# Stanford-ILIAD/PantheonRL

Measured on AMD Instinct MI355X. Metric: env-steps/sec (all agents) Overcooked-simple PPO self-play, higher is better.
Workload: dtype f32; 1 GPU; OvercookedMultiEnv-v0 layout=simple, PPO self-play (two independent PPO learners per GPU), synthetic (n_envs, n_steps, obs_dim) rollouts; n_envs=1024, n_steps=128, obs_dim=62, features=62, n_logits=6, batch_size=32768, n_epochs=10, agents_per_gpu=2, parallelism=2 agent(s) per gpu x1 gpu(s) = 2 learners (single process), launch_mode=graph, gemm_mode=2, action_masks=none, rollout=scripted, rollout_requested=scripted

## Files before the change

pantheonrl_amd/csrc/ph_abi.hip:

```cpp
#include <dlfcn.h>
#include <hip/hip_runtime.h>
#include <rccl/rccl.h>

#include <atomic>
#include <chrono>
#include <cmath>
#include <cstdio>
#include <cstdint>
#include <cstring>
#include <mutex>
#include <string>
#include <vector>

#include "ph_launch.h"
#include "ph_block.h"
#include "ph_arch.h"

namespace ph {

namespace {
struct LdsGrant {
  const void* kernel;
  int device;
  std::atomic<size_t> bytes;
// ... 84 lines not shown
  size_t grad_cap = 0;
  float* blocksq = nullptr;
  size_t blocksq_cap = 0;
  float* advstats = nullptr;
  size_t advstats_cap = 0;
  float* act_stage_host = nullptr;
  float* act_stage_dev = nullptr;
  size_t act_stage_cap = 0;
  unsigned int* act_done_host = nullptr;
  unsigned int* act_done_dev = nullptr;
  unsigned int act_seq = 0;
  unsigned int* fwd_host_done = nullptr;
  int joint_reward_rule = 0;
  int wimage_zeroed_for = 0;
  size_t wimage_cap = 0;
  bool exclusive = false;
  unsigned short* wimage = nullptr;
  double* advpart = nullptr;
  size_t advpart_cap = 0;
  int* perm_idx = nullptr;
  size_t perm_idx_cap = 0;
  int* perm_phys = nullptr;
  size_t perm_phys_cap = 0;
  uint4* ximg = nullptr;
  size_t ximg_cap = 0;
  uint4* rec_pi = nullptr;
  uint4* rec_vf = nullptr;
  size_t rec_cap = 0;
  uint4* rowrec = nullptr;
  size_t rowrec_cap = 0;
  unsigned long long* step_words = nullptr;
  size_t step_words_cap = 0;
  unsigned int* step_gen = nullptr;
  float* am_buf = nullptr;
  size_t am_buf_cap = 0;
  float* adap_extra = nullptr;
  size_t adap_extra_cap = 0;
  float* adap_loss = nullptr;
  size_t adap_loss_cap = 0;
  float* scalars = nullptr;
  int* stop_flag = nullptr;
  std::vector<SpecCache> specs;
  std::vector<hipGraphExec_t> graphs;
  bool capturing = false;
  hipEvent_t ev0 = nullptr, ev1 = nullptr;
  ph_p2p* p2p_dev = nullptr;
  ph_p2p p2p_host;
  bool p2p_valid = false;
  void* comm = nullptr;
  int comm_world = 1, comm_rank = 0;
  hipEvent_t ev_grad = nullptr;
  int num_cu = 256;
  int exchange_blocks_per_cu = 0;
  unsigned long long* rng_epoch = nullptr;
  long long* prof = nullptr;
  struct ModWs {
    float* act = nullptr;
    size_t act_cap = 0;
    int* maps = nullptr;
    ph_spec spec;
    ph_modular mod;
    bool maps_valid = false;
    float* kl_sum = nullptr;
    int* scratch = nullptr;
  } mw;
};
// ... 382 lines not shown
  hipDeviceProp_t prop;
  PH_HIP(hipGetDeviceProperties(&prop, device));
  if (std::strncmp(prop.gcnArchName, "gfx950", 6) != 0)
    return fail(std::string("device is ") + prop.gcnArchName + ", this library is built for gfx950 (MI355X) only");
  ph_ctx* c = new ph_ctx();
  c->device = device;
  c->num_cu = prop.multiProcessorCount;
  if (hipMalloc((void**)&c->scalars, 4 * sizeof(float)) != hipSuccess ||
      hipMalloc((void**)&c->stop_flag, sizeof(int)) != hipSuccess) {
    delete c;
    return fail("hipMalloc(ctx scalars) failed");
  }
  (void)hipMemset(c->scalars, 0, 4 * sizeof(float));
  (void)hipMemset(c->stop_flag, 0, sizeof(int));
  (void)hipEventCreate(&c->ev0);
  (void)hipEventCreate(&c->ev1);
  *out = c;
  return 0;
}

int ph_ctx_destroy(ph_ctx* ctx) {
  DevGuard dev_guard(ctx);
  if (!ctx) return 0;
  (void)hipStreamSynchronize(ctx->stream);
  for (auto g : ctx->graphs)
    if (g) (void)hipGraphExecDestroy(g);
  for (auto& s : ctx->specs) {
    if (s.obs_off) (void)hipFree(s.obs_off);
    if (s.slab_map) (void)hipFree(s.slab_map);
    if (s.slab_map_split) (void)hipFree(s.slab_map_split);
    if (s.wimage_map) (void)hipFree(s.wimage_map);
    if (s.act_off) (void)hipFree(s.act_off);
  }
  void* ptrs[] = {ctx->wimage, ctx->mw.act, ctx->mw.maps, ctx->mw.kl_sum, ctx->mw.scratch, ctx->advpart, ctx->p2p_dev, ctx->slabs, ctx->statpart, ctx->grad, ctx->blocksq, ctx->advstats, ctx->perm_idx, ctx->perm_phys, ctx->ximg, ctx->rec_pi, ctx->rec_vf, ctx->rowrec, ctx->step_words, ctx->step_gen, ctx->scalars, ctx->stop_flag,
                  ctx->adap_extra, ctx->adap_loss, ctx->am_buf};
  for (void* p : ptrs)
    if (p) (void)hipFree(p);
  if (ctx->act_stage_host) (void)hipHostFree(ctx->act_stage_host);
  if (ctx->act_done_host) (void)hipHostFree(ctx->act_done_host);
  if (ctx->ev0) (void)hipEventDestroy(ctx->ev0);
  if (ctx->ev1) (void)hipEventDestroy(ctx->ev1);
  if (ctx->ev_grad) (void)hipEventDestroy(ctx->ev_grad);
  (void)ph_comm_destroy(ctx);
  delete ctx;
  return 0;
}

int ph_ctx_set_joint_reward_rule(ph_ctx* ctx, int rule) {
  if (!ctx) return fail("null ctx");
  if (rule != PH_JOINT_MATCH_BONUS && rule != PH_JOINT_RPS) return fail("ph_ctx_set_joint_reward_rule: unknown rule");
  ctx->joint_reward_rule = rule;
  return 0;
}

int ph_ctx_set_stream(ph_ctx* ctx, void* hip_stream) {
  DevGuard dev_guard(ctx);
  if (!ctx) return fail("null ctx");
  ctx->stream = (hipStream_t)hip_stream;
  return 0;
}

int ph_ctx_sync(ph_ctx* ctx) {
  DevGuard dev_guard(ctx);
  if (!ctx) return fail("null ctx");
  PH_HIP(hipStreamSynchronize(ctx->stream));
  return 0;
}
// ... 1279 lines not shown
    ctx->rec_cap = n_rec;
  }
  PH_HIP(ph::launch_obs_planes(rb->observations, (int)rows, nd.D, nd.F, ph::grad_fast_fold(nd) ? 1 : 0, ctx->ximg, rb->advantages,
                               rb->log_probs, rb->actions, rb->returns, rb->values, ctx->rowrec, ctx->stream));
  return 0;
}
void fill_adv_records(ph::AdvStatArgs& aa, const ph_ctx* ctx, const ph::NetDims& nd, const ph_rollout* rb) {
  aa.rec_pi_out = nd.split == 1 ? ctx->rec_pi : nullptr;
  aa.rec_vf_out = nd.split == 1 ? ctx->rec_vf : nullptr;
  aa.rowrec = (nd.split == 1 && rb->advantages && rb->log_probs && rb->actions && rb->returns && rb->values) ? ctx->rowrec : nullptr;
  aa.rb_logp = rb->log_probs;
  aa.rb_act = rb->actions;
  aa.rb_ret = rb->returns;
  aa.rb_val = rb->values;
}


void select_gemm(ph::NetDims& nd, int gemm_mode) {
  nd.split = (gemm_mode == 2 && nd.slab_map_split != nullptr) ? nd.split_kind : 0;
  if (nd.split) nd.slab_map = nd.slab_map_split;
}

int slab_len_of(const ph::NetDims& nd) { return nd.split ? nd.slab_len_split : (nd.slab_map ? 2 * ph::RS_NET : nd.lay.P); }

int ensure_train_ws(ph_ctx* ctx, int P, int slab_len, int nwg_max, int n_mb_total, size_t n_idx = 0, size_t n_phys = 0) {
  if (n_phys && ensure(ctx, ctx->perm_phys, ctx->perm_phys_cap, n_phys)) return 1;
  if (ensure(ctx, ctx->slabs, ctx->slabs_cap, (size_t)nwg_max * slab_len)) return 1;
  if (ensure(ctx, ctx->statpart, ctx->statpart_cap, (size_t)2 * nwg_max * ph::NSTATP)) return 1;
  if (ensure(ctx, ctx->grad, ctx->grad_cap, (size_t)P)) return 1;
  if (ensure(ctx, ctx->blocksq, ctx->blocksq_cap, (size_t)ph::reduce_blocks(slab_len))) return 1;
  if (ensure(ctx, ctx->advstats, ctx->advstats_cap, (size_t)n_mb_total * 2)) return 1;
  if (ensure(ctx, ctx->advpart, ctx->advpart_cap, (size_t)n_mb_total * 2 * ph::ADV_SPLIT)) return 1;
  if (n_idx && ensure(ctx, ctx->perm_idx, ctx->perm_idx_cap, n_idx)) return 1;
  const size_t n_words = (size_t)ph::reduce_blocks(slab_len) + 1;
  if (n_words > ctx->step_words_cap) {
    if (ensure(ctx, ctx->step_words, ctx->step_words_cap, n_words)) return 1;
    PH_HIP(hipMemsetAsync(ctx->step_words, 0, n_words * sizeof(unsigned long long), ctx->stream));
  }
  if (!ctx->step_gen) {
    if (ctx->capturing) return fail("workspace would grow inside graph capture: run the same call once outside capture first");
    PH_HIP(hipMalloc((void**)&ctx->step_gen, 4 * sizeof(unsigned int)));
    PH_HIP(hipMemsetAsync(ctx->step_gen, 0, 4 * sizeof(unsigned int), ctx->stream));
  }
  return 0;
}

bool step_fused_wanted(const ph_ctx* ctx, int slab_len, bool alone) {
  return alone && ctx->exclusive && ctx->step_words && ctx->step_gen &&
         ph::step_fused_fits(ph::reduce_blocks(slab_len), slab_len, ctx->num_cu);
}

}

namespace {

struct TrainPlan {
  int alone = 1;
  ph_ctx* ctx;
  ph::NetDims nd;
  const ph_opt_state* opt;
  const ph_rollout* rb;
  const ph_ppo_hyper* hp;
  const int* perms;
  unsigned long long perm_seed;
  float* stats;
  int n_epochs, batch_size, gemm_mode, N, n_mb, P;
  uint32_t hb;
  const ph_adap_loss* adap = nullptr;
  bool arch = false;
  ph::ArchDims arch_dims;
};

int adap_check(ph_ctx* ctx, const ph::NetDims& nd, const ph_adap_loss* ad, const char* who) {
  const std::string w(who);
  if (nd.obs_kind != PH_SPACE_BOX) return fail(w + ": the context term needs Box observations (observation ++ context)");
  if (ad->context_size <= 0 || ad->context_size >= nd.F) return fail(w + ": context_size must be in (0, observation length)");
  if (ad->num_context_samples < 2 || ad->num_context_samples > ph::ADAP_ROWS)
    return fail(w + ": num_context_samples must be in [2, 16]");
  if (ad->num_state_samples <= 0) return fail(w + ": num_state_samples must be positive");
  if (ad->sampler < PH_CTX_L2 || ad->sampler > PH_CTX_NATURAL_NUMBERS) return fail(w + ": unknown context sampler");
  if (ad->sampler == PH_CTX_NATURAL_NUMBERS && ad->context_size != 1)
    return fail(w + ": the natural_numbers sampler draws (num, 1) contexts: context_size must be 1");
// ... 117 lines not shown
  g.perm_seed = t.perm_seed;
  g.perm_epoch = w.ep;
  g.epoch = ctx->rng_epoch;
  g.mb_start = w.start;
  g.nb = w.nb;
  g.advstats = ctx->advstats + 2 * (size_t)mbi;
  g.ntiles = pl.ntiles;
  *pl_out = pl;
  if (t.arch) PH_HIP(ph::launch_arch_grad(g, t.arch_dims, pl.nwg, t.gemm_mode, ctx->stream));
  else PH_HIP(ph::launch_ppo_grad(g, pl.nwg, t.gemm_mode, ctx->stream));
  return 0;
}

void fill_step_args(const TrainPlan& t, int mbi, const MbPlan& pl, ph::ReduceArgs& r, ph::AdamArgs& ad) {
  ph_ctx* ctx = t.ctx;
  float* stats_out = t.stats ? t.stats + (size_t)mbi * PH_NSTAT : nullptr;
  r = reduce_args(ctx, t.hp, t.opt, t.P, slab_len_of(t.nd), t.nd.slab_map, pl.nwg, pl.nb, ctx->grad, stats_out);
  r.wide = t.alone && ctx->exclusive;
  ad = adam_args(ctx, t.hp, t.opt, t.P, slab_len_of(t.nd), stats_out, t.nd.split ? ctx->wimage : nullptr, t.nd.wimage_map);
}

int train_launch_step(const TrainPlan& t, int mbi, const MbPlan& pl) {
  ph_ctx* ctx = t.ctx;
  hipStream_t s = ctx->stream;
  ph::ReduceArgs r;
  ph::AdamArgs ad;
  fill_step_args(t, mbi, pl, r, ad);
  if (t.adap) {
    const MbWalk w = minibatch_walk(ctx, t.perms, t.N, t.n_mb, t.batch_size, mbi);
    if (adap_launch(ctx, t.nd, t.opt->params, t.rb, t.adap, w.idx, w.nb, mbi, &r)) return 1;
  }
  if (step_fused_wanted(ctx, slab_len_of(t.nd), t.alone != 0)) {
    PH_HIP(ph::launch_ppo_step(r, ad, ctx->step_words, ctx->step_gen, ctx->step_gen + 1, STEP_WAIT_TICKS, s));
  } else {
    PH_HIP(ph::launch_ppo_reduce(r, s));
    PH_HIP(ph::launch_ppo_adam(ad, s));
  }
  return 0;
}

}

namespace {
int train_run(const char* who, ph_ctx* ctx, const ph_spec* spec, const ph_opt_state* opt, const ph_rollout* rb,
              const ph_ppo_hyper* hp, int n_epochs, int batch_size, const int* perms, unsigned long long perm_seed, float* stats,
              int gemm_mode, const ph_adap_loss* adap, const ph_arch* arch = nullptr) {
  TrainPlan t;
  if (train_prepare(who, t, ctx, spec, opt, rb, hp, n_epochs, batch_size, perms, perm_seed, stats, gemm_mode, adap != nullptr, arch))
    return 1;
  if (adap && t.nd.gauss) return fail("ph_adap_train: the context term is written for the categorical heads");
  if (adap && adap_check(ctx, t.nd, adap, "ph_adap_train")) return 1;
  t.adap = adap;
  for (int mbi = 0; mbi < n_epochs * t.n_mb; ++mbi) {
    MbPlan pl;
    if (train_launch_grad(t, mbi, &pl)) return 1;
    if (train_launch_step(t, mbi, pl)) return 1;
  }
  return 0;
}
}

int ph_ppo_train(ph_ctx* ctx, const ph_spec* spec, const ph_opt_state* opt, const ph_rollout* rb,
                 const ph_ppo_hyper* hp, int n_epochs, int batch_size, const int* perms,
                 unsigned long long perm_seed, float* stats, int gemm_mode) {
  DevGuard dev_guard(ctx);
  return train_run("ph_ppo_train", ctx, spec, opt, rb, hp, n_epochs, batch_size, perms, perm_seed, stats, gemm_mode, nullptr);
// ... 1041 lines not shown
```

pantheonrl_amd/csrc/ph_launch.h:

```cpp
#pragma once
#include "ph_device.h"

namespace ph {

__host__ __device__ inline unsigned p2p_stamp32(unsigned long long epoch, int T, int t) {
  return (unsigned)(epoch * (unsigned long long)T + (unsigned long long)t + 1ull);
}

__device__ __forceinline__ void p2p_note_timeout(unsigned long long* error, int kind, int t, unsigned long long index,
                                                 unsigned long long want, unsigned long long seen) {
  if (atomicAdd(error, 1ull) == 0ull) {
    error[1] = (unsigned long long)(unsigned)kind | ((unsigned long long)(unsigned)(t & 0xffffff) << 8) | (index << 32);
    error[2] = want;
    error[3] = seen;
  }
}

__device__ __forceinline__ void poll_backoff(int& polls) {
  if (polls < 16) __builtin_amdgcn_s_sleep(2);
  else if (polls < 64) __builtin_amdgcn_s_sleep(16);
  else __builtin_amdgcn_s_sleep(127);
  ++polls;
}

// ... 168 lines not shown
  const float* statpart;
  int nstatpart;
  float* stats_out;
  int nb;
  float ent_coef, vf_coef, target_kl;
  int* stop_flag;
  int* step;
  float* scalars;
  const float* extra = nullptr;
  int n_extra = 0, extra_len = 0, extra_cut = 0, extra_lo = 0, extra_hi = 0;
  const float* extra_loss = nullptr;
  float extra_norm = 0.f;
  float extra_coef = 0.f;
  float* extra_loss_out = nullptr;
  int wide = 0;
};

struct AdamArgs {
  float* params;
  float* m;
  float* v;
  const float* grad;
  const float* blocksq;
  int nblk, P;
  const int* step;
  const float* scalars;
  int* stop_flag;
  float lr, beta1, beta2, eps, max_norm;
  float* stats_out;
  unsigned short* wimage;
  const int* wimage_map;
};

struct StepArgs {
  ReduceArgs r;
  AdamArgs ad;
  unsigned long long* words = nullptr;
  unsigned int* gen = nullptr;
  unsigned long long timeout = 0;
  unsigned int* sweep_error = nullptr;
};

size_t fwd_lds_bytes(int R, int Lp);
size_t grad_lds_bytes(int R, int Lp, int onehot_D, int nchunk);
hipError_t launch_policy_fwd(const FwdArgs& a, int gemm_mode, hipStream_t s);
hipError_t launch_policy_fwd_multi(const FwdMulti& m, int n_agents, hipStream_t s);
hipError_t launch_fix_illegal(int* actions, const unsigned char* mask, int n, int L, hipStream_t s);
hipError_t launch_gae(const float* rew, const float* val, const float* es, const float* lv, const float* dn, float* adv,
                      float* ret, int T, int E, double gamma, double lam, int mode, hipStream_t s);
hipError_t launch_buffer_add(float* d_obs, float* d_act, float* d_rew, float* d_es, float* d_val, float* d_lp,
                             const float* obs, const float* act, const float* es, const float* val, const float* lp,
                             int E, int D, int A, hipStream_t s);
hipError_t launch_buffer_compact(const ph_rollout& src, const ph_rollout& dst, const int* cols, int n, int D, int A,
                                 hipStream_t s);
hipError_t launch_reward_add_ragged(float* rewards, const int* pos_env, const float* reward, const unsigned char* mask,
                                    int T, int E, hipStream_t s);
hipError_t launch_ragged_advance(int* pos_env, const unsigned char* mask, int T, int E, hipStream_t s);
hipError_t launch_liar_obs(const int* hands, const int* history, const int* nmoves, const unsigned char* is_ego,
                           const unsigned char* active, float* obs_out, int n, hipStream_t s);
hipError_t launch_liar_reset(int* hands, int* history, int* nmoves, const unsigned char* reset_mask,
                             unsigned char* ego_first, unsigned long long seed, unsigned long long counter,
                             const unsigned long long* epoch, float probegostart, int n, hipStream_t s);
hipError_t launch_reward_add(float* rew_row, const float* reward, const unsigned char* env_mask, int E, hipStream_t s);
hipError_t launch_reward_add_const(float* rew_row, float reward, int E, hipStream_t s);
hipError_t launch_reward_add_joint(float* rew_row, const float* base, const int* joint, int E, int n_seats, int seat,
                                   const int* partner_seat, float bonus, int rule, hipStream_t s);
hipError_t launch_framestack_push(float* stack, const float* obs, const unsigned char* reset_mask,
                                  const float* default_obs, int n, int D, int nf, hipStream_t s);
hipError_t launch_roundrobin_env_step(const int* joint, int* partnerid, const float* base, const float* done, float* reward_out,
                                      int* alt_action_out, float* next_block, int block_ld, int n_partners, float bonus, int n,
                                      hipStream_t s);
hipError_t launch_rps_step(const int* ego_act, const int* alt_act, float* ego_rew, float* alt_rew, int n, hipStream_t s);
hipError_t launch_liar_step(const int* hands, int* history, int* nmoves, const int* actions, const unsigned char* is_ego,
// ... 117 lines not shown
  const int* actions;
  int* act_dst;
};
hipError_t launch_rr_send_block(const RRSend& a, int n_partners, hipStream_t s);
hipError_t launch_rr_env_step(const RREnvStep& a, hipStream_t s);
hipError_t launch_rr_partner_pre(const RRPartnerStep& a, hipStream_t s);
hipError_t launch_rr_partner_post(const RRPartnerStep& a, hipStream_t s);
constexpr int RS_NET = 8960;
constexpr int RS_W2 = 0, RS_W1 = 4096, RS_B1 = 8192, RS_B2 = 8256, RS_HW = 8320, RS_HB = 8832;
bool grad_fast_eligible(const NetDims& nd);
bool grad_uses_reg_slabs(const NetDims& nd);
bool grad_fast_fold(const NetDims& nd);
void grad_slab_map(const ph_layout& lay, int* map , bool fold);
void grad_plan(const NetDims& nd, int nb, int num_cu, int* ntiles, int* nwg);
hipError_t launch_ppo_grad_fast(const GradArgs& a, int nwg, int gemm_mode, hipStream_t s);
bool grad_split_eligible(const NetDims& nd);
constexpr int WIMG_PLANE = 64 * 8;
constexpr int WIMG_ELEMS = 2 * 4 * 3 * 2 * 3 * WIMG_PLANE;
void grad_weight_image_map(const ph_layout& lay, bool fold, int* map );
hipError_t launch_weight_image(const float* params, unsigned short* image, const int* map, int P, hipStream_t s);
hipError_t launch_weight_image_check(const float* params, const unsigned short* image, const int* map, int P, int* mismatches,
                                     hipStream_t s);
void grad_slab_map_split(const ph_layout& lay, int* map , bool fold);
hipError_t launch_ppo_grad_split(const GradArgs& a, int nwg, hipStream_t s);
hipError_t launch_adv_stats(const AdvStatArgs& a, int n_total, hipStream_t s);
constexpr int XIMG_ROW_U4 = 24;
hipError_t launch_obs_planes(const float* obs, int n, int D, int F, int fold, uint4* image, const float* adv, const float* logp,
                             const float* act, const float* ret, const float* val, uint4* rowrec, hipStream_t s);
hipError_t launch_ppo_reduce(const ReduceArgs& a, hipStream_t s);
int reduce_blocks(int slab_len);
bool step_fused_fits(int nblk, int slab_len, int num_cu);
hipError_t launch_ppo_step(const ReduceArgs& r, const AdamArgs& ad, unsigned long long* words, unsigned int* gen,
                           unsigned int* sweep_error, unsigned long long timeout, hipStream_t st);
hipError_t launch_ppo_adam(const AdamArgs& a, hipStream_t s);
bool grad_split_oh_eligible(const NetDims& nd);
int grad_split_oh_slab_len(const NetDims& nd);
int grad_split_oh_wimage_elems(const NetDims& nd);
void grad_weight_image_map_oh(const ph_layout& lay, int nch, int* map );
void grad_slab_map_split_oh(const ph_layout& lay, int nch, int* map );
hipError_t launch_ppo_grad_split_oh(const GradArgs& a, int nwg, hipStream_t s);
hipError_t launch_set_int(int* p, int v, hipStream_t s);
size_t bc_train_lds_bytes(int F, int L, int P, int A);
hipError_t launch_bc_train(const NetDims& nd, const ph_bc_layout& lay, float* params, float* adam_m, float* adam_v, int* step,
                           const float* obs, const float* acts, const int* order, int N, int batch, int n_epochs,
                           int max_batches, const ph_bc_hyper& hp, float* stats, hipStream_t s);
hipError_t launch_bc_forward(const NetDims& nd, const ph_bc_layout& lay, const float* params, const float* obs, int n,
                             const unsigned char* mask, const float* uniforms, const float* given, uint64_t seed,
                             uint64_t counter, int deterministic, int* act_i32, float* values, float* logp, float* entropy,
                             float* logits, hipStream_t s);
hipError_t launch_epoch_advance(unsigned long long* p, hipStream_t s);

struct TowerArgs {
  int nb, ntiles;
  const float* x;
  int x_ld;
  int F;
  const int* obs_off;
  const int* idx;
  int T, E;
  const float *W1, *b1, *W2, *b2, *hW, *hb;
  int head;
  int L;
  float* h2_out;
  float* head_out;
  const float* dhead;
  const float* ext0;
// ... 66 lines not shown
```

pantheonrl_amd/csrc/ph_ppo.hip:

```cpp
#include "ph_launch.h"
#include "ph_split.h"
#include "ph_step.h"

namespace ph {


template <int N>
__device__ __forceinline__ float lds_colsum(const float* p, int stride, float s) {
#pragma unroll
  for (int r0 = 0; r0 < N; r0 += 16) {
    float t[16];
#pragma unroll
    for (int i = 0; i < 16; ++i) t[i] = p[(r0 + i) * stride];
    __builtin_amdgcn_sched_barrier(0);
#pragma unroll
    for (int i = 0; i < 16; ++i) s += t[i];
  }
  return s;
}
template <int N>
__device__ __forceinline__ float lds_coldot(const float* p, int stride, const float* q, int qstride, float s) {
#pragma unroll
  for (int r0 = 0; r0 < N; r0 += 16) {
    float t[16], u[16];
// ... 931 lines not shown
int reduce_blocks(int slab_len) { return (slab_len + RED_PARAMS - 1) / RED_PARAMS; }
static int reduce_vec(int slab_len, int exclusive) { return (slab_len % 4 == 0 && exclusive) ? 4 : (slab_len % 2 == 0 ? 2 : 1); }
bool step_fused_fits(int nblk, int slab_len, int num_cu) {
  if (nblk + 1 > 64 * 16) return false;
  static int per_cu[3] = {-1, -1, -1};
  const int vec = reduce_vec(slab_len, 1);
  int& v = per_cu[vec == 4 ? 2 : vec - 1];
  if (v < 0) {
    int api = 0;
    const void* fn = vec == 4 ? (const void*)ppo_step_kernel<4> : vec == 2 ? (const void*)ppo_step_kernel<2> : (const void*)ppo_step_kernel<1>;
    hipError_t e = hipOccupancyMaxActiveBlocksPerMultiprocessor(&api, fn, RED_PARAMS * 4, 0);
    v = (e == hipSuccess && api > 1) ? api - 1 : 0;
  }
  return (long long)v * num_cu >= (long long)nblk + 1;
}
hipError_t launch_ppo_step(const ReduceArgs& r, const AdamArgs& ad, unsigned long long* words, unsigned int* gen,
                           unsigned int* sweep_error, unsigned long long timeout, hipStream_t st) {
  StepArgs s;
  s.r = r;
  s.ad = ad;
  s.words = words;
  s.gen = gen;
  s.timeout = timeout;
  s.sweep_error = sweep_error;
  const int nblk = reduce_blocks(r.slab_len);
  if ((unsigned long long)r.nslab * (unsigned long long)r.slab_len * sizeof(float) >= (1ull << 32)) return hipErrorInvalidValue;
  switch (reduce_vec(r.slab_len, 1)) {
    case 4: hipLaunchKernelGGL(ppo_step_kernel<4>, dim3(nblk + 1), dim3(RED_PARAMS * 4), 0, st, s); break;
    case 2: hipLaunchKernelGGL(ppo_step_kernel<2>, dim3(nblk + 1), dim3(RED_PARAMS * 4), 0, st, s); break;
    default: hipLaunchKernelGGL(ppo_step_kernel<1>, dim3(nblk + 1), dim3(RED_PARAMS * 4), 0, st, s); break;
  }
  return hipGetLastError();
}
hipError_t launch_ppo_reduce(const ReduceArgs& a, hipStream_t s) {
  const dim3 grid(reduce_blocks(a.slab_len) + 1), block(RED_PARAMS * 4);
  if ((unsigned long long)a.nslab * (unsigned long long)a.slab_len * sizeof(float) >= (1ull << 32)) return hipErrorInvalidValue;
  switch (reduce_vec(a.slab_len, a.wide)) {
    case 4: hipLaunchKernelGGL(ppo_reduce_kernel<4>, grid, block, 0, s, a); break;
    case 2: hipLaunchKernelGGL(ppo_reduce_kernel<2>, grid, block, 0, s, a); break;
    default: hipLaunchKernelGGL(ppo_reduce_kernel<1>, grid, block, 0, s, a); break;
  }
  return hipGetLastError();
}

__global__ __launch_bounds__(256) void ppo_adam_kernel(AdamArgs a) {
  __shared__ float sh[4];
  __shared__ AdamScalars ks;
  const int tid = threadIdx.x;
  const int p = blockIdx.x * blockDim.x + tid;
  const bool live = p < a.P;
  float gr = 0.f, m0 = 0.f, v0 = 0.f, p0 = 0.f;
  int i0 = -1, i1 = -1;
  if (live) {
    gr = a.grad[p];
    m0 = a.m[p];
    v0 = a.v[p];
    p0 = a.params[p];
    if (a.wimage) {
      i0 = a.wimage_map[2 * p];
      i1 = a.wimage_map[2 * p + 1];
    }
  }
  if (a.scalars[1] == 0.f) {
    if (blockIdx.x == 0 && tid == 0 && a.scalars[2] != 0.f) *a.stop_flag = 1;
    return;
  }
  const int step = (tid == 0) ? *a.step : 0;
  float q = 0.f;
  {
    float x[4];
    for (int k0 = tid; k0 < a.nblk; k0 += 4 * 256) {
#pragma unroll
      for (int u = 0; u < 4; ++u) x[u] = (k0 + 256 * u < a.nblk) ? a.blocksq[k0 + 256 * u] : 0.f;
#pragma unroll
      for (int u = 0; u < 4; ++u)
        if (k0 + 256 * u < a.nblk) q += x[u];
    }
  }
  for (int off = 32; off > 0; off >>= 1) q += __shfl_down(q, off, 64);
  if ((tid & 63) == 0) sh[tid >> 6] = q;
  __syncthreads();
  if (tid == 0) {
    const float total = sqrtf((sh[0] + sh[1]) + (sh[2] + sh[3]));
    ks = adam_scalars(total, a.max_norm, step, a.lr, a.beta1, a.beta2);
    if (blockIdx.x == 0 && a.stats_out) a.stats_out[6] = total;
  }
  __syncthreads();
  if (!live) return;
  const AdamScalars k = ks;
  float m, v;
  const float pn = adam_apply(gr, k, a.beta1, a.beta2, a.eps, m0, v0, p0, &m, &v);
  a.m[p] = m;
  a.v[p] = v;
  a.params[p] = pn;
  if (a.wimage) wimage_put_at(a.wimage, i0, i1, pn);
}

__global__ __launch_bounds__(256) void weight_image_kernel(const float* params, unsigned short* image, const int* map, int P) {
  const int p = blockIdx.x * blockDim.x + threadIdx.x;
  if (p < P) wimage_put(image, map, p, params[p]);
}
__global__ __launch_bounds__(256) void weight_image_check_kernel(const float* params, const unsigned short* image, const int* map, int P,
                                                                 int* mismatches) {
  const int p = blockIdx.x * blockDim.x + threadIdx.x;
  if (p >= P) return;
  __bf16 h, m, l;
  split1(params[p], h, m, l);
  const unsigned short want[3] = {__builtin_bit_cast(unsigned short, h), __builtin_bit_cast(unsigned short, m),
                                  __builtin_bit_cast(unsigned short, l)};
  int bad = 0;
  for (int k = 0; k < 2; ++k) {
    const int pos = map[2 * p + k];
    if (pos < 0) continue;
    for (int q = 0; q < 3; ++q) bad += image[pos + q * WIMG_PLANE] != want[q];
  }
  if (bad) atomicAdd(mismatches, bad);
}
// ... 27 lines not shown
```

pantheonrl_amd/csrc/ph_step.h:

```cpp
#pragma once
#include "ph_launch.h"
#include "ph_split.h"

namespace ph {

constexpr int RED_PARAMS = 64, RED_SUB = 16, RED_SHIFT = 6;

struct AdamScalars {
  float coef, ss, bc2s;
};
__device__ __forceinline__ AdamScalars adam_scalars(float total_norm, float max_norm, int step, float lr, float beta1, float beta2) {
  AdamScalars k;
  const float cc = max_norm / (total_norm + 1e-6f);
  k.coef = cc < 1.0f ? cc : 1.0f;
  const double t = (double)step;
  const double bc1 = 1.0 - pow((double)beta1, t);
  const double bc2 = 1.0 - pow((double)beta2, t);
  k.ss = (float)((double)lr / bc1);
  k.bc2s = (float)sqrt(bc2);
  return k;
}
__device__ __forceinline__ float adam_apply(float grad, const AdamScalars& k, float beta1, float beta2, float eps, float m0, float v0,
                                            float p0, float* m_out, float* v_out) {
#pragma clang fp contract(off)
// ... 188 lines not shown
    stop = (a.target_kl >= 0.f) && (kl > 1.5f * a.target_kl);
    if (bump_step && !stop && a.step) *a.step += 1;
    a.scalars[0] = kl;
    a.scalars[1] = stop ? 0.f : 1.f;
    a.scalars[2] = stop ? 1.f : 0.f;
    if (a.stats_out) {
      a.stats_out[0] = pl_;
      a.stats_out[1] = vl;
      a.stats_out[2] = el;
      a.stats_out[3] = cf;
      a.stats_out[4] = kl;
      a.stats_out[5] = pl_ + a.ent_coef * el + a.vf_coef * vl;
      a.stats_out[6] = 0.f;
      a.stats_out[7] = stop ? 0.f : 1.f;
    }
    if (a.n_extra > 0) {
      float raw = 0.f;
      for (int k0 = 0; k0 < a.n_extra; k0 += 16) {
        float x[16];
#pragma unroll
        for (int u = 0; u < 16; ++u) x[u] = (k0 + u < a.n_extra) ? a.extra_loss[k0 + u] : 0.f;
#pragma unroll
        for (int u = 0; u < 16; ++u)
          if (k0 + u < a.n_extra) raw += x[u];
      }
      raw *= a.extra_norm;
      if (a.extra_loss_out) *a.extra_loss_out = raw;
      if (a.stats_out) a.stats_out[5] += a.extra_coef * raw;
    }
  }
  return stop;
}

__device__ __forceinline__ void step_finish(const StepArgs& s, int nblk, unsigned tag, int step_new, int lane, bool first, float g,
                                            int dst, float m0, float v0, float p0, int i0, int i1) {
  const ReduceArgs& a = s.r;
  const AdamArgs& ad = s.ad;
  AdamScalars k = adam_scalars(0.f, ad.max_norm, step_new, ad.lr, ad.beta1, ad.beta2);
  constexpr int MAXW = 16;
  float qv[MAXW];
  bool ok = false;
  const long long t0 = wall_clock64();
  while (true) {
    bool all = true;
#pragma unroll
    for (int i = 0; i < MAXW; ++i) {
      const int k = lane + 64 * i;
      qv[i] = 0.f;
      if (k <= nblk) {
        const unsigned long long w = __hip_atomic_load(s.words + k, __ATOMIC_RELAXED, __HIP_MEMORY_SCOPE_AGENT);
        all = all && ((unsigned)(w >> 32) == tag);
        qv[i] = __uint_as_float((unsigned)w);
      }
    }
    if (__all(all)) { ok = true; break; }
    if ((unsigned long long)(wall_clock64() - t0) > s.timeout) break;
    __builtin_amdgcn_s_sleep(4);
  }
  if (!ok) {
    if (lane == 0) {
      atomicAdd(s.sweep_error, 1u);
      if (first && a.stats_out) a.stats_out[7] = -1.f;
    }
    return;
  }
  int stop_i = 0;
#pragma unroll
  for (int i = 0; i < MAXW; ++i)
    if (lane + 64 * i == nblk) stop_i = __float_as_int(qv[i]) & 1;
  const bool stop = __any(stop_i != 0);
  float shv[4];
#pragma unroll
  for (int v = 0; v < 4; ++v) {
    float q = 0.f;
#pragma unroll
    for (int i = v; i < MAXW; i += 4)
      if (lane + 64 * i < nblk) q += qv[i];
    for (int off = 32; off > 0; off >>= 1) q += __shfl_down(q, off, 64);
    shv[v] = __shfl(q, 0, 64);
  }
  const float total = sqrtf((shv[0] + shv[1]) + (shv[2] + shv[3]));
  if (first && lane == 0) {
    if (!stop && ad.step) *const_cast<int*>(ad.step) = step_new;
    if (stop) *a.stop_flag = 1;
    *s.gen = tag;
    if (!stop && a.stats_out) a.stats_out[6] = total;
  }
  if (stop || dst < 0) return;
  {
    const float cc = ad.max_norm / (total + 1e-6f);
    k.coef = cc < 1.0f ? cc : 1.0f;
  }
  const int p = dst;
  float m, v;
  const float pn = adam_apply(g, k, ad.beta1, ad.beta2, ad.eps, m0, v0, p0, &m, &v);
  ad.m[p] = m;
  ad.v[p] = v;
  ad.params[p] = pn;
  if (ad.wimage) wimage_put_at(ad.wimage, i0, i1, pn);
}


__device__ __forceinline__ void step_stopped(const ReduceArgs& a) {
  const int tid = threadIdx.x;
  if (tid < PH_NSTAT && a.stats_out) a.stats_out[tid] = 0.f;
  if (tid == 0) {
    a.scalars[1] = 0.f;
    a.scalars[2] = 0.f;
  }
}
__device__ __forceinline__ bool step_refused(const ReduceArgs& a, int blk, int stopped, unsigned err) {
  if (err != 0u) {
    if (blk == 0 && threadIdx.x == 0 && a.stats_out) a.stats_out[7] = -1.f;
    return true;
// ... 13 lines not shown
  if (blk == nblk) {
    if (step_refused(a, blk, stopped, err)) return;
    const bool stop = reduce_statistics<COH>(a, part, means, false);
    if (tid == 0)
      __hip_atomic_store(s.words + nblk, ((unsigned long long)tag << 32) | (stop ? 1ull : 0ull), __ATOMIC_RELAXED, __HIP_MEMORY_SCOPE_AGENT);
    return;
  }
  const int dst = reduce_dst(a, blk);
  float m0 = 0.f, v0 = 0.f, p0 = 0.f;
  int i0 = -1, i1 = -1;
  if (dst >= 0) {
    m0 = ad.m[dst];
    v0 = ad.v[dst];
    p0 = ad.params[dst];
    if (ad.wimage) {
      i0 = ad.wimage_map[2 * dst];
      i1 = ad.wimage_map[2 * dst + 1];
    }
  }
  const float g = reduce_positions<VEC, COH>(a, gsum, dst, blk);
  if (step_refused(a, blk, stopped, err)) return;
  if (tid < 64) {
    float q = g * g;
    for (int off = 32; off > 0; off >>= 1) q += __shfl_down(q, off, 64);
    if (tid == 0)
      __hip_atomic_store(s.words + blk, ((unsigned long long)tag << 32) | (unsigned long long)__float_as_uint(q), __ATOMIC_RELAXED,
                         __HIP_MEMORY_SCOPE_AGENT);
  }
  if (tid >= 64) return;
  step_finish(s, nblk, tag, step_new, tid, blk == 0, g, dst, m0, v0, p0, i0, i1);
}


__host__ __device__ inline int reduce_blocks_of(int slab_len) { return (slab_len + RED_PARAMS - 1) / RED_PARAMS; }

}
```

pantheonrl_amd/ppo.py:

```python
from __future__ import annotations

import ctypes as C
import os
import io
import json
import time
import zipfile
from collections import deque
from typing import Sequence, Any, Dict, Optional, Tuple

import numpy as np
import torch as th

from . import _native as nat
from . import spaces as sp
from .logger import Logger, configure_logger

HID = nat.PH_HIDDEN


def _require_cuda(device) -> th.device:
    dev = th.device("cuda" if device in (None, "auto") else device)
    if dev.type != "cuda":
        raise nat.NativeError(
# ... 637 lines not shown
        prog = getattr(self, "_current_progress_remaining", 1.0)
        h.learning_rate, h.clip_range = self._schedule(self.learning_rate, prog), self._schedule(self.clip_range, prog)
        h.clip_range_vf = -1.0 if self.clip_range_vf is None else self._schedule(self.clip_range_vf, prog)
        h.ent_coef, h.vf_coef, h.max_grad_norm = float(self.ent_coef), float(self.vf_coef), float(self.max_grad_norm)
        h.target_kl = -1.0 if self.target_kl is None else float(self.target_kl)
        h.normalize_advantage = int(bool(self.normalize_advantage))
        h.adam_beta1, h.adam_beta2, h.adam_eps = 0.9, 0.999, 1e-5
        return h

    def train(self, perms: Optional[np.ndarray] = None, sync_stats: bool = True) -> None:
        rb, pol = self.rollout_buffer, self.policy
        N = rb.buffer_size * rb.n_envs
        n_mb = (N + self.batch_size - 1) // self.batch_size
        perm_t = None
        if perms is None and not self.device_permutations:
            perms = np.stack([np.random.permutation(N) for _ in range(self.n_epochs)])
        if perms is not None:
            perm_t = th.as_tensor(np.ascontiguousarray(perms, dtype=np.int32)).to(self.device)
            assert perm_t.shape == (self.n_epochs, N)
        stats = getattr(self, "_stats_dev", None)
        if stats is None or stats.shape[0] != self.n_epochs * n_mb:
            stats = th.zeros((self.n_epochs * n_mb, nat.PH_NSTAT), dtype=th.float32, device=self.device)
        opt = nat.PhOptState()
        opt.params, opt.adam_m, opt.adam_v = pol.params.data_ptr(), pol.adam_m.data_ptr(), pol.adam_v.data_ptr()
        opt.step = pol.opt_step.data_ptr()
        hp = self.hyper()
        pol._bind()
        self.permutation_seed += 1
        self._train_native(pol, opt, rb, hp, perm_t, stats)
        self._n_updates += self.n_epochs
        self._stats_dev = stats
        if sync_stats:
            st = stats.cpu().numpy()
            expired = pol.ctx.step_errors() if pol.ctx.exclusive_hint else 0
            seen, self._step_errors_seen = getattr(self, "_step_errors_seen", 0), expired
            if (st[:, 7] < 0).any() or expired > seen:
                raise nat.NativeError("PPO.train: a wait of the one-launch optimizer step expired (is the device really this "
                                      "learner's alone? ph_set_exclusive_device): the update was applied only in part")
            self.last_train_stats = st
            applied = st[:, 7] > 0
            n_used = int(applied.sum()) + (1 if not applied.all() else 0)
            used = st[:max(n_used, 1)]
            lg = self.logger
            ret = rb.returns.flatten()
            var_y = float(ret.var(unbiased=False))
            ev = float("nan") if var_y == 0 else 1.0 - float((ret - rb.values.flatten()).var(unbiased=False)) / var_y
            lg.record("train/explained_variance", ev)
            lg.record("train/entropy_loss", float(used[:, 2].mean()))
            lg.record("train/policy_gradient_loss", float(used[:, 0].mean()))
            lg.record("train/value_loss", float(used[:, 1].mean()))
            lg.record("train/approx_kl", float(used[((len(used) - 1) // n_mb) * n_mb:, 4].mean()))
            lg.record("train/clip_fraction", float(used[:, 3].mean()))
            lg.record("train/loss", float(used[-1, 5]))
            lg.record("train/n_updates", self._n_updates, exclude="tensorboard")
            lg.record("train/clip_range", float(hp.clip_range))
            lg.record("train/learning_rate", float(hp.learning_rate))

    def _train_native(self, pol, opt, rb, hp, perm_t, stats) -> None:
        if isinstance(pol, ArchActorCriticPolicy):
            nat.check(pol.ctx.lib.ph_arch_train(pol.ctx.handle, C.byref(pol.spec), C.byref(pol.arch), C.byref(opt),
                                                C.byref(rb.c_struct()), C.byref(hp), int(self.n_epochs), int(self.batch_size),
                                                nat.ptr(perm_t), int(self.permutation_seed), stats.data_ptr(), int(pol.gemm_mode)))
            return
        if not getattr(pol, "gaussian_head", False):
            require_mlp_kernels(pol, "PPO.train")
        nat.check(pol.ctx.lib.ph_ppo_train(pol.ctx.handle, C.byref(pol.spec), C.byref(opt), C.byref(rb.c_struct()),
                                           C.byref(hp), int(self.n_epochs), int(self.batch_size), nat.ptr(perm_t),
                                           int(self.permutation_seed), stats.data_ptr(), int(pol.gemm_mode)))

    def _train_call(self, keep: list) -> "nat.PhTrainCall":
        rb, pol = self.rollout_buffer, self.policy
# ... 221 lines not shown
```

Measured before the change: 119.2 million agent-steps/s.

## Fuse gradient reduce and Adam into one ticket-ordered launch for shared devices

Adds a single-launch optimizer step for the case where the fused step is not allowed, i.e. two learners share the GPU. Blocks take tickets from an atomic counter: ticket 0 computes statistics, the next tickets reduce gradient slabs and publish tagged per-parameter entries, and the remaining tickets spin until their entries and the norm words are ready, then apply Adam. Ordering by ticket means waiting blocks only depend on blocks that were already scheduled, so it is safe without exclusive residency. This saves a kernel launch and the inter-kernel gap per minibatch, at the cost of spin-wait polling, extra atomics and a per-parameter entries buffer.

```diff
diff --git a/pantheonrl_amd/csrc/ph_abi.hip b/pantheonrl_amd/csrc/ph_abi.hip
--- a/pantheonrl_amd/csrc/ph_abi.hip
+++ b/pantheonrl_amd/csrc/ph_abi.hip
@@ -140,6 +140,8 @@
   unsigned long long* step_words = nullptr;
   size_t step_words_cap = 0;
   unsigned int* step_gen = nullptr;
+  unsigned long long* step_entries = nullptr;
+  size_t step_entries_cap = 0;
   float* am_buf = nullptr;
   size_t am_buf_cap = 0;
   float* adap_extra = nullptr;
@@ -588,7 +590,7 @@
     if (s.wimage_map) (void)hipFree(s.wimage_map);
     if (s.act_off) (void)hipFree(s.act_off);
   }
-  void* ptrs[] = {ctx->wimage, ctx->mw.act, ctx->mw.maps, ctx->mw.kl_sum, ctx->mw.scratch, ctx->advpart, ctx->p2p_dev, ctx->slabs, ctx->statpart, ctx->grad, ctx->blocksq, ctx->advstats, ctx->perm_idx, ctx->perm_phys, ctx->ximg, ctx->rec_pi, ctx->rec_vf, ctx->rowrec, ctx->step_words, ctx->step_gen, ctx->scalars, ctx->stop_flag,
+  void* ptrs[] = {ctx->wimage, ctx->mw.act, ctx->mw.maps, ctx->mw.kl_sum, ctx->mw.scratch, ctx->advpart, ctx->p2p_dev, ctx->slabs, ctx->statpart, ctx->grad, ctx->blocksq, ctx->advstats, ctx->perm_idx, ctx->perm_phys, ctx->ximg, ctx->rec_pi, ctx->rec_vf, ctx->rowrec, ctx->step_words, ctx->step_entries, ctx->step_gen, ctx->scalars, ctx->stop_flag,
                   ctx->adap_extra, ctx->adap_loss, ctx->am_buf};
   for (void* p : ptrs)
     if (p) (void)hipFree(p);
@@ -1934,10 +1936,14 @@
   if (ensure(ctx, ctx->advstats, ctx->advstats_cap, (size_t)n_mb_total * 2)) return 1;
   if (ensure(ctx, ctx->advpart, ctx->advpart_cap, (size_t)n_mb_total * 2 * ph::ADV_SPLIT)) return 1;
   if (n_idx && ensure(ctx, ctx->perm_idx, ctx->perm_idx_cap, n_idx)) return 1;
-  const size_t n_words = (size_t)ph::reduce_blocks(slab_len) + 1;
+  const size_t n_words = std::max((size_t)ph::reduce_blocks(slab_len) + 1, (size_t)64 * ph::STEP_MAXW);
   if (n_words > ctx->step_words_cap) {
     if (ensure(ctx, ctx->step_words, ctx->step_words_cap, n_words)) return 1;
     PH_HIP(hipMemsetAsync(ctx->step_words, 0, n_words * sizeof(unsigned long long), ctx->stream));
+  }
+  if ((size_t)P > ctx->step_entries_cap) {
+    if (ensure(ctx, ctx->step_entries, ctx->step_entries_cap, (size_t)P)) return 1;
+    PH_HIP(hipMemsetAsync(ctx->step_entries, 0, (size_t)P * sizeof(unsigned long long), ctx->stream));
   }
   if (!ctx->step_gen) {
     if (ctx->capturing) return fail("workspace would grow inside graph capture: run the same call once outside capture first");
@@ -1950,6 +1956,14 @@
 bool step_fused_wanted(const ph_ctx* ctx, int slab_len, bool alone) {
   return alone && ctx->exclusive && ctx->step_words && ctx->step_gen &&
          ph::step_fused_fits(ph::reduce_blocks(slab_len), slab_len, ctx->num_cu);
+}
+
+bool step_ordered_wanted(const ph_ctx* ctx, int slab_len, int P) {
+  static const bool on = [] {
+    const char* e = getenv("PH_STEP_ORDERED");
+    return !(e && e[0] == '0');
+  }();
+  return on && ctx->step_words && ctx->step_entries && ctx->step_gen && ph::step_ordered_fits(ph::reduce_blocks(slab_len), P);
 }
 
 }
@@ -2133,6 +2147,9 @@
   }
   if (step_fused_wanted(ctx, slab_len_of(t.nd), t.alone != 0)) {
     PH_HIP(ph::launch_ppo_step(r, ad, ctx->step_words, ctx->step_gen, ctx->step_gen + 1, STEP_WAIT_TICKS, s));
+  } else if (!r.wide && ad.step && step_ordered_wanted(ctx, slab_len_of(t.nd), t.P)) {
+    PH_HIP(ph::launch_ppo_step_ordered(r, ad, ctx->step_words, ctx->step_entries, ctx->step_gen, ctx->step_gen + 1, ctx->step_gen + 2,
+                                       STEP_WAIT_TICKS, s));
   } else {
     PH_HIP(ph::launch_ppo_reduce(r, s));
     PH_HIP(ph::launch_ppo_adam(ad, s));
diff --git a/pantheonrl_amd/csrc/ph_launch.h b/pantheonrl_amd/csrc/ph_launch.h
--- a/pantheonrl_amd/csrc/ph_launch.h
+++ b/pantheonrl_amd/csrc/ph_launch.h
@@ -224,6 +224,7 @@
   const int* wimage_map;
 };
 
+constexpr int STEP_MAXW = 16;
 struct StepArgs {
   ReduceArgs r;
   AdamArgs ad;
@@ -231,6 +232,8 @@
   unsigned int* gen = nullptr;
   unsigned long long timeout = 0;
   unsigned int* sweep_error = nullptr;
+  unsigned long long* entries = nullptr;
+  unsigned int* counters = nullptr;
 };
 
 size_t fwd_lds_bytes(int R, int Lp);
@@ -414,6 +417,10 @@
 bool step_fused_fits(int nblk, int slab_len, int num_cu);
 hipError_t launch_ppo_step(const ReduceArgs& r, const AdamArgs& ad, unsigned long long* words, unsigned int* gen,
                            unsigned int* sweep_error, unsigned long long timeout, hipStream_t st);
+bool step_ordered_fits(int nblk, int P);
+hipError_t launch_ppo_step_ordered(const ReduceArgs& r, const AdamArgs& ad, unsigned long long* words, unsigned long long* entries,
+                                   unsigned int* gen, unsigned int* sweep_error, unsigned int* counters, unsigned long long timeout,
+                                   hipStream_t st);
 hipError_t launch_ppo_adam(const AdamArgs& a, hipStream_t s);
 bool grad_split_oh_eligible(const NetDims& nd);
 int grad_split_oh_slab_len(const NetDims& nd);
diff --git a/pantheonrl_amd/csrc/ph_ppo.hip b/pantheonrl_amd/csrc/ph_ppo.hip
--- a/pantheonrl_amd/csrc/ph_ppo.hip
+++ b/pantheonrl_amd/csrc/ph_ppo.hip
@@ -987,6 +987,63 @@
   }
   return hipGetLastError();
 }
+__device__ __forceinline__ const StepArgs& ordered_args() {
+  auto kp = __builtin_amdgcn_kernarg_segment_ptr();
+  asm volatile("" : "+s"(kp));
+  return *(const StepArgs*)kp;
+}
+template <int VEC>
+__global__ __launch_bounds__(RED_PARAMS * 4) void ppo_step_ordered_kernel(StepArgs s, int nblk, int nadam) {
+  __shared__ float lds_union[4 * RED_PARAMS];
+  __shared__ float means[NSTATP];
+  float (*gsum)[RED_PARAMS] = reinterpret_cast<float (*)[RED_PARAMS]>(lds_union);
+  float (*part)[NSTATP] = reinterpret_cast<float (*)[NSTATP]>(lds_union);
+  unsigned* sh = reinterpret_cast<unsigned*>(lds_union);
+  const int tid = threadIdx.x;
+  const int stopped = *s.r.stop_flag;
+  const unsigned tag = *s.gen + 1u;
+  const int step_new = *s.ad.step + 1;
+  const unsigned err = *s.sweep_error;
+  if (tid == 0) {
+    sh[0] = 0u;
+    reinterpret_cast<unsigned*>(means)[0] = __hip_atomic_fetch_add(s.counters, 1u, __ATOMIC_RELAXED, __HIP_MEMORY_SCOPE_AGENT);
+  }
+  __syncthreads();
+  const int ticket = __builtin_amdgcn_readfirstlane((int)reinterpret_cast<const unsigned*>(means)[0]);
+  unsigned verdict = 0u;
+  if (ticket == 0) {
+    verdict = ordered_statistics(ordered_args(), nblk, tag, part, means, stopped, err);
+  } else if (ticket <= nblk) {
+    ordered_reduce<VEC>(ordered_args(), ticket - 1, tag, gsum, stopped, err);
+  } else {
+    verdict = ordered_adam(ordered_args(), nblk, (ticket - nblk - 1) * ORD_ADAM_LANES, ticket == nblk + 1, tag, step_new, sh, stopped, err);
+  }
+  if (tid == 0) ordered_finish(ordered_args(), (unsigned)(1 + nblk + nadam), verdict, tag, step_new, stopped, err);
+}
+bool step_ordered_fits(int nblk, int P) {
+  const long long nadam = ((long long)P + ORD_ADAM_LANES - 1) / ORD_ADAM_LANES;
+  return nblk + 1 <= 64 * STEP_MAXW && nadam < (1 << 14) && 1 + nblk + nadam <= (long long)ORD_COUNT;
+}
+hipError_t launch_ppo_step_ordered(const ReduceArgs& r, const AdamArgs& ad, unsigned long long* words, unsigned long long* entries,
+                                   unsigned int* gen, unsigned int* sweep_error, unsigned int* counters, unsigned long long timeout,
+                                   hipStream_t st) {
+  StepArgs s;
+  s.r = r;
+  s.ad = ad;
+  s.words = words;
+  s.gen = gen;
+  s.timeout = timeout;
+  s.sweep_error = sweep_error;
+  s.entries = entries;
+  s.counters = counters;
+  const int nblk = reduce_blocks(r.slab_len), nadam = (ad.P + ORD_ADAM_LANES - 1) / ORD_ADAM_LANES;
+  if (!step_ordered_fits(nblk, ad.P) || !ad.step) return hipErrorInvalidValue;
+  if ((unsigned long long)r.nslab * (unsigned long long)r.slab_len * sizeof(float) >= (1ull << 32)) return hipErrorInvalidValue;
+  const dim3 grid(1 + nblk + nadam), block(RED_PARAMS * 4);
+  if (reduce_vec(r.slab_len, 0) == 2) hipLaunchKernelGGL(ppo_step_ordered_kernel<2>, grid, block, 0, st, s, nblk, nadam);
+  else hipLaunchKernelGGL(ppo_step_ordered_kernel<1>, grid, block, 0, st, s, nblk, nadam);
+  return hipGetLastError();
+}
 hipError_t launch_ppo_reduce(const ReduceArgs& a, hipStream_t s) {
   const dim3 grid(reduce_blocks(a.slab_len) + 1), block(RED_PARAMS * 4);
   if ((unsigned long long)a.nslab * (unsigned long long)a.slab_len * sizeof(float) >= (1ull << 32)) return hipErrorInvalidValue;
@@ -1020,7 +1077,8 @@
     if (blockIdx.x == 0 && tid == 0 && a.scalars[2] != 0.f) *a.stop_flag = 1;
     return;
   }
-  const int step = (tid == 0) ? *a.step : 0;
+  AdamScalars k0{};
+  if (tid == 0) k0 = adam_scalars(0.f, a.max_norm, *a.step, a.lr, a.beta1, a.beta2);
   float q = 0.f;
   {
     float x[4];
@@ -1037,7 +1095,9 @@
   __syncthreads();
   if (tid == 0) {
     const float total = sqrtf((sh[0] + sh[1]) + (sh[2] + sh[3]));
-    ks = adam_scalars(total, a.max_norm, step, a.lr, a.beta1, a.beta2);
+    const float cc = a.max_norm / (total + 1e-6f);
+    k0.coef = cc < 1.0f ? cc : 1.0f;
+    ks = k0;
     if (blockIdx.x == 0 && a.stats_out) a.stats_out[6] = total;
   }
   __syncthreads();
diff --git a/pantheonrl_amd/csrc/ph_step.h b/pantheonrl_amd/csrc/ph_step.h
--- a/pantheonrl_amd/csrc/ph_step.h
+++ b/pantheonrl_amd/csrc/ph_step.h
@@ -244,27 +244,75 @@
   return stop;
 }
 
+__device__ __forceinline__ bool step_words_pass(const unsigned long long* words, int nblk, unsigned tag, int lane, float (&qv)[STEP_MAXW]) {
+  bool all = true;
+#pragma unroll
+  for (int i = 0; i < STEP_MAXW; ++i) {
+    const int k = lane + 64 * i;
+    qv[i] = 0.f;
+    if (k <= nblk) {
+      const unsigned long long w = __hip_atomic_load(words + k, __ATOMIC_RELAXED, __HIP_MEMORY_SCOPE_AGENT);
+      all = all && ((unsigned)(w >> 32) == tag);
+      qv[i] = __uint_as_float((unsigned)w);
+    }
+  }
+  return all;
+}
+__device__ __forceinline__ bool step_words_pass_lean(const unsigned long long* words, int nblk, unsigned tag, int lane,
+                                                     float (&qv)[STEP_MAXW]) {
+  constexpr int H = STEP_MAXW / 2;
+  const int need = lane <= nblk ? (nblk - lane) / 64 + 1 : 0;
+  int got = 0;
+#pragma unroll
+  for (int h = 0; h < 2; ++h) {
+    if (h == 1 && nblk < 64 * H) {
+#pragma unroll
+      for (int i = H; i < STEP_MAXW; ++i) qv[i] = 0.f;
+      break;
+    }
+    if (h == 1) __builtin_amdgcn_sched_barrier(0);
+    unsigned off = (unsigned)((lane + 64 * H * h) * sizeof(unsigned long long));
+    asm volatile("" : "+v"(off));
+    const unsigned long long* base = reinterpret_cast<const unsigned long long*>(reinterpret_cast<const char*>(words) + off);
+    unsigned long long w[H];
+#pragma unroll
+    for (int i = 0; i < H; ++i) w[i] = __hip_atomic_load(base + 64 * i, __ATOMIC_RELAXED, __HIP_MEMORY_SCOPE_AGENT);
+#pragma unroll
+    for (int i = 0; i < H; ++i) {
+      got += (unsigned)(w[i] >> 32) == tag ? 1 : 0;
+      qv[h * H + i] = __uint_as_float((unsigned)w[i]);
+    }
+  }
+  return got == need;
+}
+__device__ __forceinline__ float step_words_norm(const float (&qv)[STEP_MAXW], int nblk, int lane, bool* stop_out) {
+  int stop_i = 0;
+#pragma unroll
+  for (int i = 0; i < STEP_MAXW; ++i)
+    if (lane + 64 * i == nblk) stop_i = __float_as_int(qv[i]) & 1;
+  *stop_out = __any(stop_i != 0);
+  float shv[4];
+#pragma unroll
+  for (int v = 0; v < 4; ++v) {
+    float q = 0.f;
+#pragma unroll
+    for (int i = v; i < STEP_MAXW; i += 4)
+      if (lane + 64 * i < nblk) q += qv[i];
+    for (int off = 32; off > 0; off >>= 1) q += __shfl_down(q, off, 64);
+    shv[v] = __shfl(q, 0, 64);
+  }
+  return sqrtf((shv[0] + shv[1]) + (shv[2] + shv[3]));
+}
 __device__ __forceinline__ void step_finish(const StepArgs& s, int nblk, unsigned tag, int step_new, int lane, bool first, float g,
                                             int dst, float m0, float v0, float p0, int i0, int i1) {
   const ReduceArgs& a = s.r;
   const AdamArgs& ad = s.ad;
   AdamScalars k = adam_scalars(0.f, ad.max_norm, step_new, ad.lr, ad.beta1, ad.beta2);
-  constexpr int MAXW = 16;
-  float qv[MAXW];
+  float qv[STEP_MAXW];
   bool ok = false;
   const long long t0 = wall_clock64();
   while (true) {
-    bool all = true;
-#pragma unroll
-    for (int i = 0; i < MAXW; ++i) {
-      const int k = lane + 64 * i;
-      qv[i] = 0.f;
-      if (k <= nblk) {
-        const unsigned long long w = __hip_atomic_load(s.words + k, __ATOMIC_RELAXED, __HIP_MEMORY_SCOPE_AGENT);
-        all = all && ((unsigned)(w >> 32) == tag);
-        qv[i] = __uint_as_float((unsigned)w);
-      }
-    }
+    const bool all = step_words_pass(s.words, nblk, tag, lane, qv);
     if (__all(all)) { ok = true; break; }
     if ((unsigned long long)(wall_clock64() - t0) > s.timeout) break;
     __builtin_amdgcn_s_sleep(4);
@@ -276,22 +324,8 @@
     }
     return;
   }
-  int stop_i = 0;
-#pragma unroll
-  for (int i = 0; i < MAXW; ++i)
-    if (lane + 64 * i == nblk) stop_i = __float_as_int(qv[i]) & 1;
-  const bool stop = __any(stop_i != 0);
-  float shv[4];
-#pragma unroll
-  for (int v = 0; v < 4; ++v) {
-    float q = 0.f;
-#pragma unroll
-    for (int i = v; i < MAXW; i += 4)
-      if (lane + 64 * i < nblk) q += qv[i];
-    for (int off = 32; off > 0; off >>= 1) q += __shfl_down(q, off, 64);
-    shv[v] = __shfl(q, 0, 64);
-  }
-  const float total = sqrtf((shv[0] + shv[1]) + (shv[2] + shv[3]));
+  bool stop;
+  const float total = step_words_norm(qv, nblk, lane, &stop);
   if (first && lane == 0) {
     if (!stop && ad.step) *const_cast<int*>(ad.step) = step_new;
     if (stop) *a.stop_flag = 1;
@@ -371,6 +405,116 @@
 }
 
 
+constexpr unsigned ORD_COUNT = 0xffffu, ORD_STOP = 1u << 16, ORD_ERR = 1u << 17;
+constexpr int ORD_ADAM_LANES = 256;
+
+__device__ __forceinline__ unsigned ordered_statistics(const StepArgs& s, int nblk, unsigned tag, float (*part)[NSTATP], float* means,
+                                                       int stopped, unsigned err) {
+  if (step_refused(s.r, 0, stopped, err)) return 0u;
+  const bool stop = reduce_statistics(s.r, part, means, false);
+  if (threadIdx.x != 0) return 0u;
+  asm volatile("s_waitcnt vmcnt(0)" ::: "memory");
+  __hip_atomic_store(s.words + nblk, ((unsigned long long)tag << 32) | (stop ? 1ull : 0ull), __ATOMIC_RELAXED, __HIP_MEMORY_SCOPE_AGENT);
+  return stop ? ORD_STOP : 0u;
+}
+template <int VEC>
+__device__ __forceinline__ void ordered_reduce(const StepArgs& s, int blk, unsigned tag, float (*gsum)[RED_PARAMS], int stopped,
+                                               unsigned err) {
+  const int tid = threadIdx.x;
+  const int dst = reduce_dst(s.r, blk);
+  const float g = reduce_positions<VEC>(s.r, gsum, dst, blk);
+  if (step_refused(s.r, 1, stopped, err) || tid >= 64) return;
+  if (dst >= 0)
+    __hip_atomic_store(s.entries + dst, ((unsigned long long)tag << 32) | (unsigned long long)__float_as_uint(g), __ATOMIC_RELAXED,
+                       __HIP_MEMORY_SCOPE_AGENT);
+  float q = g * g;
+  for (int off = 32; off > 0; off >>= 1) q += __shfl_down(q, off, 64);
+  if (tid == 0)
+    __hip_atomic_store(s.words + blk, ((unsigned long long)tag << 32) | (unsigned long long)__float_as_uint(q), __ATOMIC_RELAXED,
+                       __HIP_MEMORY_SCOPE_AGENT);
+}
+__device__ __forceinline__ unsigned ordered_adam(const StepArgs& s, int nblk, int p_base, bool first, unsigned tag, int step_new,
+                                                 unsigned* sh, int stopped, unsigned err) {
+  const ReduceArgs& a = s.r;
+  const AdamArgs& ad = s.ad;
+  if (step_refused(a, 1, stopped, err)) return 0u;
+  const int tid = threadIdx.x, lane = tid & 63;
+  const int wave = __builtin_amdgcn_readfirstlane(tid >> 6);
+  const int p = p_base + tid;
+  const bool live = p < ad.P;
+  float m0 = 0.f, v0 = 0.f, p0 = 0.f;
+  int i0 = -1, i1 = -1;
+  if (live) {
+    m0 = ad.m[p];
+    v0 = ad.v[p];
+    p0 = ad.params[p];
+    if (ad.wimage) {
+      i0 = ad.wimage_map[2 * p];
+      i1 = ad.wimage_map[2 * p + 1];
+    }
+  }
+  AdamScalars k = adam_scalars(0.f, ad.max_norm, step_new, ad.lr, ad.beta1, ad.beta2);
+  float qv[STEP_MAXW];
+  const unsigned long long* ep = s.entries + (live ? p : ad.P - 1);
+  unsigned long long e;
+  bool ok = false;
+  const long long t0 = wall_clock64();
+  while (true) {
+    e = __hip_atomic_load(ep, __ATOMIC_RELAXED, __HIP_MEMORY_SCOPE_AGENT);
+    bool all = true;
+    if (wave == 0) all = step_words_pass_lean(s.words, nblk, tag, lane, qv);
+    all = all && (!live || (unsigned)(e >> 32) == tag);
+    if (__all(all)) { ok = true; break; }
+    if ((unsigned long long)(wall_clock64() - t0) > s.timeout) break;
+    __builtin_amdgcn_s_sleep(4);
+  }
+  if (!ok && lane == 0) sh[0] = 1u;
+  if (wave == 0 && ok) {
+    bool stop;
+    const float total = step_words_norm(qv, nblk, lane, &stop);
+    if (lane == 0) {
+      sh[1] = stop ? 1u : 0u;
+      sh[2] = __float_as_uint(total);
+    }
+  }
+  __syncthreads();
+  if (sh[0] != 0u) {
+    if (tid == 0) {
+      atomicAdd(s.sweep_error, 1u);
+      if (a.stats_out) a.stats_out[7] = -1.f;
+    }
+    return ORD_ERR;
+  }
+  if (sh[1] != 0u) return 0u;
+  const float total = __uint_as_float(sh[2]);
+  if (first && tid == 0 && a.stats_out) a.stats_out[6] = total;
+  if (!live) return 0u;
+  {
+    const float cc = ad.max_norm / (total + 1e-6f);
+    k.coef = cc < 1.0f ? cc : 1.0f;
+  }
+  float m, v;
+  const float pn = adam_apply(__uint_as_float((unsigned)e), k, ad.beta1, ad.beta2, ad.eps, m0, v0, p0, &m, &v);
+  ad.m[p] = m;
+  ad.v[p] = v;
+  ad.params[p] = pn;
+  if (ad.wimage) wimage_put_at(ad.wimage, i0, i1, pn);
+  return 0u;
+}
+__device__ __forceinline__ void ordered_finish(const StepArgs& s, unsigned total_blocks, unsigned verdict, unsigned tag, int step_new,
+                                               int stopped, unsigned err) {
+  const unsigned add = 1u + verdict;
+  const unsigned sum = __hip_atomic_fetch_add(s.counters + 1, add, __ATOMIC_RELAXED, __HIP_MEMORY_SCOPE_AGENT) + add;
+  if ((sum & ORD_COUNT) != total_blocks) return;
+  const bool applied = stopped == 0 && err == 0u && (sum >> 17) == 0u;
+  const bool stop = (sum & ORD_STOP) != 0u;
+  if (applied && !stop && s.ad.step) *const_cast<int*>(s.ad.step) = step_new;
+  if (applied && stop) *s.r.stop_flag = 1;
+  *s.gen = tag;
+  __hip_atomic_store(s.counters, 0u, __ATOMIC_RELAXED, __HIP_MEMORY_SCOPE_AGENT);
+  __hip_atomic_store(s.counters + 1, 0u, __ATOMIC_RELAXED, __HIP_MEMORY_SCOPE_AGENT);
+}
+
 __host__ __device__ inline int reduce_blocks_of(int slab_len) { return (slab_len + RED_PARAMS - 1) / RED_PARAMS; }
 
 }
diff --git a/pantheonrl_amd/ppo.py b/pantheonrl_amd/ppo.py
--- a/pantheonrl_amd/ppo.py
+++ b/pantheonrl_amd/ppo.py
@@ -693,11 +693,10 @@
         self._stats_dev = stats
         if sync_stats:
             st = stats.cpu().numpy()
-            expired = pol.ctx.step_errors() if pol.ctx.exclusive_hint else 0
-            seen, self._step_errors_seen = getattr(self, "_step_errors_seen", 0), expired
-            if (st[:, 7] < 0).any() or expired > seen:
-                raise nat.NativeError("PPO.train: a wait of the one-launch optimizer step expired (is the device really this "
-                                      "learner's alone? ph_set_exclusive_device): the update was applied only in part")
+            if (st[:, 7] < 0).any() or pol.ctx.step_errors() > 0:
+                raise nat.NativeError("PPO.train: a wait of the one-launch optimizer step expired: an update was applied only "
+                                      "in part and this policy's context skips every update from then on (with "
+                                      "ph_set_exclusive_device: is the device really this learner's alone?)")
             self.last_train_stats = st
             applied = st[:, 7] > 0
             n_used = int(applied.sum()) + (1 if not applied.all() else 0)
```

Result: slower. 112.5 million agent-steps/s (-5.6%).
